# stella-cv/stella_vslam

Hardware: AMD Instinct MI355X
Metric: frames/s ORB-extract+match @640x480,2k kpts (higher is better)
Workload: dtype u8

## Files before the change

stella_vslam_amd/csrc/orb_kernels.hip:

```cpp
#include "svgpu_internal.h"
#include "sv_trig.h"
#include <utility>

#pragma clang fp contract(off)

namespace {

__device__ __constant__ float c_pattern_f[1024] = {
#include "orb_pattern_i8.inc"
};

__device__ __forceinline__ int find_level(const OrbLevel* __restrict__ L, int num_levels, int idx, int OrbLevel::*first,
                                          int* local) {
    int lv = 0;
    for (int l = 0; l < num_levels; ++l) {
        const int f = L[l].*first;
        if (idx >= f) lv = l;
    }
    *local = idx - L[lv].*first;
    return lv;
}

__device__ __forceinline__ int reflect101(int p, int len) {
    if (len == 1) return 0;
// ... 732 lines not shown
            const uint32_t order = (uint32_t)cell.order_base | ((uint32_t)ly << 7) | (uint32_t)qx;
            const unsigned long long key = ((unsigned long long)(uint32_t)s << 32) | (0xFFFFFFFFu - order);
            const int kx = gx - gx0, ky = gy - gy0;
            if ((unsigned)kx < FAST_KT && (unsigned)ky < FAST_KT) atomicMax(&s_key[ky * FAST_KT + kx], key);
            else atomicMax(&K[gy * lev.grid_x + gx], key);
        }
        if (found) atomicAdd(&s_count, found);
        __syncthreads();
        if (s_count > 0) break;
        __syncthreads();
    }
    }
    if (tid < FAST_KT * FAST_KT) {
        const unsigned long long key = s_key[tid];
        if (key) atomicMax(&K[(gy0 + tid / FAST_KT) * lev.grid_x + gx0 + tid % FAST_KT], key);
    }
    }
}

__global__ __launch_bounds__(1024) void k_select(const OrbLevel* __restrict__ L, int num_levels, unsigned long long* __restrict__ keys,
                                                 int total_grid, int4* __restrict__ sel, int32_t* __restrict__ counts, int32_t* __restrict__ cellpos) {
    __shared__ int s_wave[16], s_lvcnt[SV_MAX_LEVELS];
    const int b = blockIdx.x, tid = threadIdx.x, lane = tid & 63, wave = tid >> 6;
    unsigned long long* K = keys + (size_t)b * total_grid;
    int4* S = sel + (size_t)b * total_grid;
    if (tid < SV_MAX_LEVELS) s_lvcnt[tid] = 0;
    int running = 0;
    for (int base = 0; base < total_grid; base += 1024) {
        const int idx = base + tid;
        unsigned long long key = 0;
        if (idx < total_grid) {
            key = K[idx];
            if (key) K[idx] = 0;
        }
        const unsigned long long bal = __ballot(key != 0);
        const int before = __popcll(bal & ((1ull << lane) - 1ull));
        __syncthreads();
        if (lane == 0) s_wave[wave] = __popcll(bal);
        __syncthreads();
        int woff = 0, total = 0;
#pragma unroll
        for (int k = 0; k < 16; ++k) {
            if (k < wave) woff += s_wave[k];
            total += s_wave[k];
        }
        if (cellpos && idx < total_grid) cellpos[(size_t)b * (total_grid + 1) + idx] = running + woff + before;
        if (key) {
            int lv = 0;
            while (lv + 1 < num_levels && idx >= L[lv + 1].grid_first) ++lv;
            const uint32_t order = 0xFFFFFFFFu - (uint32_t)(key & 0xFFFFFFFFu);
            const int lx = order & 127, ly = (order >> 7) & 127, cid = order >> 14;
            const int cells_x = L[lv].cells_x;
            const int ci = cid / cells_x, cj = cid - ci * cells_x;
            int4 r;
            r.x = SV_PATCH_RADIUS + cj * SV_CELL + lx;
            r.y = SV_PATCH_RADIUS + ci * SV_CELL + ly;
            r.z = lv;
            r.w = (int)(key >> 32);
            S[running + woff + before] = r;
            atomicAdd(&s_lvcnt[lv], 1);
        }
        running += total;
    }
    __syncthreads();
    if (tid < num_levels) counts[b * (1 + num_levels) + 1 + tid] = s_lvcnt[tid];
    if (tid == 0) {
        counts[b * (1 + num_levels)] = running;
        if (cellpos) cellpos[(size_t)b * (total_grid + 1) + total_grid] = running;
    }
}

__device__ __forceinline__ float dev_fast_atan2(float y, float x) {
    const float p1 = 0.9997878412794807f * (float)(180 / 3.1415926535897932384626433832795);
    const float p3 = -0.3258083974640975f * (float)(180 / 3.1415926535897932384626433832795);
    const float p5 = 0.1555786518463281f * (float)(180 / 3.1415926535897932384626433832795);
    const float p7 = -0.04432655554792128f * (float)(180 / 3.1415926535897932384626433832795);
    const float eps = (float)2.2204460492503131e-16;
    const float ax = fabsf(x), ay = fabsf(y);
    float a, c, c2;
    if (ax >= ay) {
        c = ay / (ax + eps);
        c2 = c * c;
        a = (((p7 * c2 + p5) * c2 + p3) * c2 + p1) * c;
    }
    else {
        c = ax / (ay + eps);
        c2 = c * c;
        a = 90.f - (((p7 * c2 + p5) * c2 + p3) * c2 + p1) * c;
    }
    if (x < 0) a = 180.f - a;
    if (y < 0) a = 360.f - a;
    return a;
}

__device__ __forceinline__ float dev_util_cos(float v) { return sv_util_cos(v); }
__device__ __forceinline__ float dev_util_sin(float v) { return sv_util_sin(v); }

__device__ __forceinline__ int wave_sum(int v) {
    v += __builtin_amdgcn_update_dpp(0, v, 0x111, 0xF, 0xF, false);
    v += __builtin_amdgcn_update_dpp(0, v, 0x112, 0xF, 0xF, false);
    v += __builtin_amdgcn_update_dpp(0, v, 0x114, 0xF, 0xF, false);
    v += __builtin_amdgcn_update_dpp(0, v, 0x118, 0xF, 0xF, false);
    v += __builtin_amdgcn_update_dpp(0, v, 0x142, 0xA, 0xF, false);
    v += __builtin_amdgcn_update_dpp(0, v, 0x143, 0xC, 0xF, false);
    return __builtin_amdgcn_readlane(v, 63);
}

#ifndef DESC_KPW
#define DESC_KPW 5
#endif
#define DESC_IP 32
#define DESC_BP 40
#define DESC_R 18
#define DESC_SLAB (DESC_KPW * 37 * DESC_BP + 16)
struct IcWeights {
    uint32_t w1[256], wu[256];
};
constexpr IcWeights make_ic_weights() {
    constexpr int umax[16] = {15, 15, 15, 15, 14, 14, 14, 13, 13, 12, 11, 10, 9, 8, 6, 3};
    IcWeights t{};
    for (int row = 0; row < 31; ++row)
        for (int j = 0; j < 8; ++j) {
            uint32_t w1 = 0, wu = 0;
            const int v = row - 15, av = v < 0 ? -v : v;
            for (int k = 0; k < 4; ++k) {
                const int col = 4 * j + k, u = col - 15, au = u < 0 ? -u : u;
                if (col < 31 && au <= umax[av]) {
                    w1 |= 1u << (8 * k);
                    wu |= (uint32_t)(u + 15) << (8 * k);
                }
            }
            t.w1[row * 8 + j] = w1;
            t.wu[row * 8 + j] = wu;
        }
    return t;
}
__device__ __constant__ IcWeights c_icw = make_ic_weights();

__global__ __launch_bounds__(256) void k_describe(const OrbLevel* __restrict__ L, int num_levels, const int4* __restrict__ sel,
                                                  int total_grid, const int32_t* __restrict__ counts,
                                                  const uint8_t* __restrict__ img0, size_t img0_frame_stride, int img0_pitch,
                                                  const uint8_t* __restrict__ pyr, size_t pyr_frame_bytes,
                                                  const uint8_t* __restrict__ blur, size_t blur_frame_bytes,
                                                  svgpu_keypoint* __restrict__ kps, uint8_t* __restrict__ desc, int cap, float* __restrict__ angles) {
    __shared__ __attribute__((aligned(16))) uint8_t s_slab[4][DESC_SLAB];
    int b, blk;
    xcd_frame_map(gridDim.x, gridDim.y, blk, b);
    const int lane = threadIdx.x & 63, wave = __builtin_amdgcn_readfirstlane(threadIdx.x >> 6);
    const int n = min(counts[b * (1 + num_levels)], cap);
    const int i0 = (blk * 4 + wave) * DESC_KPW;
    if (i0 >= n) return;
    uint8_t* const slab = s_slab[wave];
    float px0[4], py0[4], px1[4], py1[4];
#pragma unroll
    for (int r = 0; r < 4; ++r) {
        const float4 q = reinterpret_cast<const float4*>(c_pattern_f)[r * 64 + lane];
        px0[r] = q.x;
        py0[r] = q.y;
        px1[r] = q.z;
        py1[r] = q.w;
    }
    uint32_t w1[4], wu[4];
    int rowv[4];
#pragma unroll
    for (int m = 0; m < 4; ++m) {
        const int item = lane + 64 * m;
        w1[m] = c_icw.w1[item];
        wu[m] = c_icw.wu[item];
        rowv[m] = (item >> 3) - 15;
    }
    const int nk = min(DESC_KPW, n - i0);
    const int4* const S = sel + (size_t)b * total_grid + i0;
    const uint8_t* const I0 = img0 + (size_t)b * img0_frame_stride;
    const uint8_t* const PY = pyr + (size_t)b * pyr_frame_bytes;
    const uint8_t* const BL = blur + (size_t)b * blur_frame_bytes;
    const int part = lane & 3, prow = lane >> 2;
    const int br = lane / 5, bpart = lane - 5 * br;
    int4 sv[DESC_KPW];
#pragma unroll
    for (int kk = 0; kk < DESC_KPW; ++kk) sv[kk] = S[kk];
    const uint8_t* gi[DESC_KPW];
    const uint8_t* gbl[DESC_KPW];
    int pit_i[DESC_KPW], pit_b[DESC_KPW];
#pragma unroll
    for (int kk = 0; kk < DESC_KPW; ++kk) {
        const int lv = kk < nk ? sv[kk].z : 0;
        pit_b[kk] = L[lv].pitch;
        pit_i[kk] = lv == 0 ? img0_pitch : pit_b[kk];
        gi[kk] = (lv == 0 ? I0 : PY + L[lv].pyr_off) + (size_t)(sv[kk].y - 15) * pit_i[kk] + (sv[kk].x - 15);
        gbl[kk] = BL + L[lv].blur_off + (size_t)(sv[kk].y - DESC_R) * pit_b[kk] + (sv[kk].x - DESC_R);
    }
    uint2 vi[DESC_KPW][2];
#pragma unroll
    for (int kk = 0; kk < DESC_KPW; ++kk)
        if (kk < nk) {
#pragma unroll
            for (int h = 0; h < 2; ++h)
                if (16 * h + prow < 31) __builtin_memcpy(&vi[kk][h], gi[kk] + (__umul24(16 * h + prow, pit_i[kk]) + 8 * part), 8);
        }
#pragma unroll
    for (int kk = 0; kk < DESC_KPW; ++kk)
        if (kk < nk) {
#pragma unroll
            for (int h = 0; h < 2; ++h)
                if (16 * h + prow < 31) *reinterpret_cast<uint2*>(slab + kk * (31 * DESC_IP) + (16 * h + prow) * DESC_IP + 8 * part) = vi[kk][h];
        }
    __builtin_amdgcn_fence(__ATOMIC_RELEASE, "wavefront");
    __builtin_amdgcn_wave_barrier();
    __builtin_amdgcn_fence(__ATOMIC_ACQUIRE, "wavefront");
    uint2 vb[DESC_KPW][4];
#pragma unroll
    for (int kk = 0; kk < DESC_KPW; ++kk)
        if (kk < nk) {
#pragma unroll
            for (int h = 0; h < 4; ++h)
                if (br < 12 && 12 * h + br < 37) __builtin_memcpy(&vb[kk][h], gbl[kk] + (__umul24(12 * h + br, pit_b[kk]) + 8 * bpart), 8);
        }
    int my10 = 0, my01 = 0;
#pragma unroll
    for (int kk = 0; kk < DESC_KPW; ++kk)
        if (kk < nk) {
            int m10 = 0, m01 = 0;
#pragma unroll
            for (int m = 0; m < 4; ++m) {
                const int item = lane + 64 * m;
                const uint32_t px = item < 248 ? reinterpret_cast<const uint32_t*>(slab + kk * (31 * DESC_IP))[item] : 0u;
                const int s1 = (int)__builtin_amdgcn_udot4(px, w1[m], 0u, false), su = (int)__builtin_amdgcn_udot4(px, wu[m], 0u, false);
                m10 += su - __mul24(15, s1);
                m01 += __mul24(rowv[m], s1);
            }
            m10 = wave_sum(m10);
            m01 = wave_sum(m01);
            if (lane == kk) {
                my10 = m10;
                my01 = m01;
            }
        }
    const float angle = dev_fast_atan2((float)my01, (float)my10);
    const float rad = (float)((double)angle * 3.14159265358979323846 / 180.0);
    const float ca_l = dev_util_cos(rad), sa_l = dev_util_sin(rad);
    __builtin_amdgcn_fence(__ATOMIC_RELEASE, "wavefront");
    __builtin_amdgcn_wave_barrier();
#pragma unroll
    for (int kk = 0; kk < DESC_KPW; ++kk)
        if (kk < nk) {
#pragma unroll
            for (int h = 0; h < 4; ++h)
                if (br < 12 && 12 * h + br < 37) *reinterpret_cast<uint2*>(slab + kk * (37 * DESC_BP) + __mul24(12 * h + br, DESC_BP) + 8 * bpart) = vb[kk][h];
        }
    __builtin_amdgcn_fence(__ATOMIC_RELEASE, "wavefront");
    __builtin_amdgcn_wave_barrier();
    __builtin_amdgcn_fence(__ATOMIC_ACQUIRE, "wavefront");
#pragma unroll
    for (int kk = 0; kk < DESC_KPW; ++kk)
        if (kk < nk) {
            const float ca = __int_as_float(__builtin_amdgcn_readlane(__float_as_int(ca_l), kk));
            const float sa = __int_as_float(__builtin_amdgcn_readlane(__float_as_int(sa_l), kk));
            const uint8_t* B = slab + kk * (37 * DESC_BP) + DESC_R * DESC_BP + DESC_R;
            unsigned long long bits[4];
#pragma unroll
            for (int r = 0; r < 4; ++r) {
                const float x0 = px0[r], y0 = py0[r], x1 = px1[r], y1 = py1[r];
                constexpr float RN = 12582912.0f;
                constexpr int RK = 0x400000 * DESC_BP + 0x4B400000;
                typedef float f32x2 __attribute__((ext_vector_type(2)));
                const f32x2 sc = {sa, ca}, cs = {ca, -sa}, rn = {RN, RN};
                const f32x2 q0 = (f32x2{x0, x0} * sc + f32x2{y0, y0} * cs) + rn;
                const f32x2 q1 = (f32x2{x1, x1} * sc + f32x2{y1, y1} * cs) + rn;
                const int r0 = __float_as_int(q0.x), c0 = __float_as_int(q0.y);
                const int r1 = __float_as_int(q1.x), c1 = __float_as_int(q1.y);
                const int a = B[__mul24(r0, DESC_BP) + c0 - RK];
                const int bb = B[__mul24(r1, DESC_BP) + c1 - RK];
                bits[r] = __builtin_amdgcn_ballot_w64(a < bb);
            }
            uint8_t* D = desc + ((size_t)b * cap + i0 + kk) * 32;
            if (lane < 4) reinterpret_cast<unsigned long long*>(D)[lane] = lane == 0 ? bits[0] : lane == 1 ? bits[1] : lane == 2 ? bits[2] : bits[3];
        }
    if (lane < nk) {
        const int4 s = S[lane];
        const int lv = s.z;
        svgpu_keypoint k;
        k.x = (float)s.x;
        k.y = (float)s.y;
        if (lv != 0) {
            k.x = k.x * L[lv].scale;
            k.y = k.y * L[lv].scale;
        }
        k.size = L[lv].kp_size;
        k.angle = angle;
        k.response = (float)s.w;
        k.octave = lv;
        k.class_id = -1;
        kps[(size_t)b * cap + i0 + lane] = k;
        if (angles) angles[(size_t)b * cap + i0 + lane] = angle;
    }
}


#ifndef DB_THREADS
#define DB_THREADS 512
#endif
#define DB_WAVES (DB_THREADS / 64)
#define DB_MAX_KP 128
struct IcWeights3 {
    uint32_t w1[256], wu[256], wv[256];
};
constexpr IcWeights3 make_ic_weights3() {
    constexpr int umax[16] = {15, 15, 15, 15, 14, 14, 14, 13, 13, 12, 11, 10, 9, 8, 6, 3};
    IcWeights3 t{};
    for (int row = 0; row < 31; ++row)
        for (int j = 0; j < 8; ++j) {
            uint32_t w1 = 0, wu = 0, wv = 0;
            const int v = row - 15, av = v < 0 ? -v : v;
            for (int k = 0; k < 4; ++k) {
                const int col = 4 * j + k, u = col - 15, au = u < 0 ? -u : u;
                if (col < 31 && au <= umax[av]) {
                    w1 |= 1u << (8 * k);
                    wu |= (uint32_t)(u + 15) << (8 * k);
                    wv |= (uint32_t)row << (8 * k);
                }
            }
            t.w1[row * 8 + j] = w1;
            t.wu[row * 8 + j] = wu;
            t.wv[row * 8 + j] = wv;
        }
    return t;
}
__device__ __constant__ IcWeights3 c_icw3 = make_ic_weights3();

template <int LANE>
__device__ __forceinline__ void sv_writelane8(uint32_t& lo, uint32_t& hi, const unsigned long long (&m)[4]) {
    asm("s_nop 1\n\tv_writelane_b32 %0, %2, %10\n\tv_writelane_b32 %1, %3, %10\n\tv_writelane_b32 %0, %4, %11\n\tv_writelane_b32 %1, %5, %11\n\t"
        "v_writelane_b32 %0, %6, %12\n\tv_writelane_b32 %1, %7, %12\n\tv_writelane_b32 %0, %8, %13\n\tv_writelane_b32 %1, %9, %13"
        : "+v"(lo), "+v"(hi)
        : "s"((uint32_t)m[0]), "s"((uint32_t)(m[0] >> 32)), "s"((uint32_t)m[1]), "s"((uint32_t)(m[1] >> 32)), "s"((uint32_t)m[2]), "s"((uint32_t)(m[2] >> 32)),
          "s"((uint32_t)m[3]), "s"((uint32_t)(m[3] >> 32)), "n"(LANE), "n"(LANE + 1), "n"(LANE + 2), "n"(LANE + 3));
}

__device__ __forceinline__ void db_stage_rows(const uint8_t* img, int gp, int y0, int nrows, int cpr, uint32_t lds0, int lane, int wave) {
    const int rpi = 64 / cpr;
    const int rsub = lane / cpr, csub = lane - rsub * cpr;
    const uint32_t voff = (uint32_t)(rsub * gp + csub * 16);
    const int groups = (nrows + rpi - 1) / rpi;
    const unsigned long long base = (unsigned long long)(uintptr_t)(img + (size_t)y0 * gp);
    if (rsub < rpi)
        for (int g = wave; g < groups; g += DB_WAVES)
            if (g * rpi + rsub < nrows) sv_glds16(base + (unsigned long long)(g * rpi) * (unsigned)gp, voff, lds0 + (uint32_t)(g * rpi * cpr) * 16);
}
__device__ __forceinline__ void db_stage_rows_wide(const uint8_t* img, int gp, int y0, int nrows, int cpr, uint32_t lds0, int lane, int wave) {
    const int total = nrows * cpr;
    int q = wave * 64 + lane;
    int row = q / cpr, c = q - row * cpr;
    const int drow = (DB_WAVES * 64) / cpr, dc = (DB_WAVES * 64) - drow * cpr;
    const unsigned long long base = (unsigned long long)(uintptr_t)(img + (size_t)y0 * gp);
    uint32_t dst = lds0 + wave * 1024;
    for (int i = wave * 64; i < total; i += DB_WAVES * 64) {
        if (q < total) sv_glds16(base, (uint32_t)(row * gp + c * 16), dst);
        q += DB_WAVES * 64;
        row += drow;
        c += dc;
        if (c >= cpr) {
            c -= cpr;
            ++row;
        }
        dst += DB_WAVES * 1024;
    }
}

__global__ __launch_bounds__(DB_THREADS) void k_describe_bands(const OrbLevel* __restrict__ L, int num_levels, const DescBand* __restrict__ bands, int num_bands,
                                                               const int4* __restrict__ sel, int total_grid, const int32_t* __restrict__ cellpos,
                                                               const int32_t* __restrict__ counts,
                                                               const uint8_t* __restrict__ img0, size_t img0_frame_stride, int img0_pitch,
                                                               const uint8_t* __restrict__ pyr, size_t pyr_frame_bytes,
                                                               const uint8_t* __restrict__ blur, size_t blur_frame_bytes,
                                                               svgpu_keypoint* __restrict__ kps, uint8_t* __restrict__ desc, int cap, float* __restrict__ angles) {
    extern __shared__ __attribute__((aligned(16))) uint8_t s_band[];
    int b, bi;
    xcd_frame_map(gridDim.x, gridDim.y, bi, b);
    const DescBand bd = bands[bi];
    const int tid = threadIdx.x, lane = tid & 63, wave = __builtin_amdgcn_readfirstlane(tid >> 6);
    const int32_t* const P = cellpos + (size_t)b * (total_grid + 1);
    const int n = min(counts[b * (1 + num_levels)], cap);
    const int p0 = P[bd.cell0], nkp = min(P[bd.cell1], n) - p0;
    if (nkp <= 0) return;
    const int lv = bd.lv, lp = bd.lp, cpr = lp >> 4;
    int2* const s_xy = reinterpret_cast<int2*>(s_band + bd.img_bytes);
    int2* const s_aux = s_xy + DB_MAX_KP;
    const uint32_t lds0 = __builtin_amdgcn_readfirstlane((uint32_t)(uintptr_t)(const __attribute__((address_space(3))) uint8_t*)s_band);
    const int4* const S = sel + (size_t)b * total_grid + p0;
    int4 sv = make_int4(0, 0, 0, 0);
    if (tid < nkp) {
        sv = S[tid];
        s_xy[tid] = make_int2(sv.x, sv.y);
    }
    uint32_t w1[4], wu[4], wv[4];
#pragma unroll
    for (int m = 0; m < 4; ++m) {
        const int item = lane + 64 * m;
        w1[m] = c_icw3.w1[item];
        wu[m] = c_icw3.wu[item];
        wv[m] = c_icw3.wv[item];
    }
    float px0[4], py0[4], px1[4], py1[4];
#pragma unroll
    for (int r = 0; r < 4; ++r) {
        const float4 q = reinterpret_cast<const float4*>(c_pattern_f)[r * 64 + lane];
        px0[r] = q.x;
        py0[r] = q.y;
        px1[r] = q.z;
        py1[r] = q.w;
    }
    {
        const uint8_t* img = lv == 0 ? img0 + (size_t)b * img0_frame_stride : pyr + (size_t)b * pyr_frame_bytes + L[lv].pyr_off;
        asm volatile("s_waitcnt vmcnt(0) lgkmcnt(0)" ::: "memory");
        if (cpr <= 64) db_stage_rows(img, lv == 0 ? img0_pitch : L[lv].pitch, bd.yu0, bd.nru, cpr, lds0, lane, wave);
        else db_stage_rows_wide(img, lv == 0 ? img0_pitch : L[lv].pitch, bd.yu0, bd.nru, cpr, lds0, lane, wave);
        asm volatile("s_waitcnt vmcnt(0)" ::: "memory");
    }
    __syncthreads();
    {
        const int lane_off = (lane >> 3) * lp + 4 * (lane & 7), step = 8 * lp;
        for (int j = wave; j < nkp; j += DB_WAVES) {
            const int2 xy = s_xy[j];
            const int x = __builtin_amdgcn_readfirstlane(xy.x), y = __builtin_amdgcn_readfirstlane(xy.y);
            const int org = (y - 15 - bd.yu0) * lp + (x - 15);
            const uint32_t* U = reinterpret_cast<const uint32_t*>(s_band + ((org & ~3) + lane_off));
            const uint32_t sh = (org & 3) * 8;
            uint32_t s1 = 0, su = 0, sw = 0;
#pragma unroll
            for (int m = 0; m < 4; ++m) {
                const uint32_t lo = U[m * (step >> 2)], hi = U[m * (step >> 2) + 1];
                const uint32_t px = __builtin_amdgcn_alignbit(hi, lo, sh);
                s1 = __builtin_amdgcn_udot4(px, w1[m], s1, false);
                su = __builtin_amdgcn_udot4(px, wu[m], su, false);
                sw = __builtin_amdgcn_udot4(px, wv[m], sw, false);
            }
            const int m10 = wave_sum((int)su - __mul24(15, (int)s1)), m01 = wave_sum((int)sw - __mul24(15, (int)s1));
            if (lane == 0) s_aux[j] = make_int2(m10, m01);
        }
    }
    __syncthreads();
    if (cpr <= 64) db_stage_rows(blur + (size_t)b * blur_frame_bytes + L[lv].blur_off, L[lv].pitch, bd.yb0, bd.nrb, cpr, lds0, lane, wave);
    else db_stage_rows_wide(blur + (size_t)b * blur_frame_bytes + L[lv].blur_off, L[lv].pitch, bd.yb0, bd.nrb, cpr, lds0, lane, wave);
    if (tid < nkp) {
        const int2 mm = s_aux[tid];
        const float angle = dev_fast_atan2((float)mm.y, (float)mm.x);
        const float rad = (float)((double)angle * 3.14159265358979323846 / 180.0);
        s_aux[tid] = make_int2(__float_as_int(dev_util_cos(rad)), __float_as_int(dev_util_sin(rad)));
        svgpu_keypoint k;
        k.x = (float)sv.x;
        k.y = (float)sv.y;
        if (lv != 0) {
            k.x = k.x * L[lv].scale;
            k.y = k.y * L[lv].scale;
        }
        k.size = L[lv].kp_size;
        k.angle = angle;
        k.response = (float)sv.w;
        k.octave = lv;
        k.class_id = -1;
        kps[(size_t)b * cap + p0 + tid] = k;
        if (angles) angles[(size_t)b * cap + p0 + tid] = angle;
    }
    asm volatile("s_waitcnt vmcnt(0)" ::: "memory");
    __syncthreads();
    {
        constexpr float RN = 12582912.0f;
        const int rk = 0x400000 * lp + 0x4B400000;
        for (int j = wave; j < nkp; j += DB_WAVES) {
            const int2 xy = s_xy[j], cs2 = s_aux[j];
            const int x = __builtin_amdgcn_readfirstlane(xy.x), y = __builtin_amdgcn_readfirstlane(xy.y);
            const float ca = __int_as_float(__builtin_amdgcn_readfirstlane(cs2.x)), sa = __int_as_float(__builtin_amdgcn_readfirstlane(cs2.y));
            const uint8_t* B = s_band + ((y - bd.yb0) * lp + x - rk);
            unsigned long long bits[4];
#pragma unroll
            for (int r = 0; r < 4; ++r) {
                typedef float f32x2 __attribute__((ext_vector_type(2)));
                const f32x2 sc = {sa, ca}, cs = {ca, -sa}, rn = {RN, RN};
                const f32x2 q0 = (f32x2{px0[r], px0[r]} * sc + f32x2{py0[r], py0[r]} * cs) + rn;
                const f32x2 q1 = (f32x2{px1[r], px1[r]} * sc + f32x2{py1[r], py1[r]} * cs) + rn;
                const int a = B[__mul24(__float_as_int(q0.x), lp) + __float_as_int(q0.y)];
                const int bb = B[__mul24(__float_as_int(q1.x), lp) + __float_as_int(q1.y)];
                bits[r] = __builtin_amdgcn_ballot_w64(a < bb);
            }
            uint32_t d_lo = 0, d_hi = 0;
            sv_writelane8<0>(d_lo, d_hi, bits);
            if (lane < 4) reinterpret_cast<uint2*>(desc + ((size_t)b * cap + p0 + j) * 32)[lane] = make_uint2(d_lo, d_hi);
        }
    }
}

}

hipError_t sv_pyramid_prepare() {
    return sv_allow_dynamic_lds(reinterpret_cast<const void*>(k_pyramid_lds), SV_PYR_LDS_MAX);
}
void sv_launch_pyramid(hipStream_t s, const OrbFrames& F, const OrbLaunch& plan, const int2* band_rows, int bands, size_t lds_bytes, const short* xofs,
                       const short2* xa, const short2* yofs, const short2* yb, const uint32_t* xg, const short4* yrow) {
    if (plan.pyramid_lds)
        hipLaunchKernelGGL(k_pyramid_lds, dim3(bands, F.batch), dim3(PYR_THREADS), lds_bytes, s, F.levels, F.num_levels, band_rows, bands, F.img0,
                           F.img0_frame_stride, F.img0_pitch, F.pyr, F.pyr_frame_bytes, xg, yrow);
    else
        hipLaunchKernelGGL(k_pyramid, dim3(bands, F.batch), dim3(PYR_THREADS), 0, s, F.levels, F.num_levels, band_rows, F.img0, F.img0_frame_stride,
                           F.img0_pitch, F.pyr, F.pyr_frame_bytes, xofs, xa, yofs, yb);
}

void sv_launch_blur(hipStream_t s, const OrbFrames& F, const OrbLaunch& plan, int total_tiles, int total_bands) {
    const dim3 grid(total_tiles, F.batch), block(256);
    if (!plan.blur_bands) {
        hipLaunchKernelGGL(k_blur<BLUR_ROWS_SMALL>, grid, block, 0, s, F.levels, F.num_levels, F.img0, F.img0_frame_stride, F.img0_pitch, F.pyr,
                           F.pyr_frame_bytes, F.blur, F.blur_frame_bytes);
        if (plan.need_gather)
            hipLaunchKernelGGL(k_blur_gather<BLUR_ROWS_SMALL>, grid, block, 0, s, F.levels, F.num_levels, F.img0, F.img0_frame_stride, F.img0_pitch, F.pyr,
                               F.pyr_frame_bytes, F.blur, F.blur_frame_bytes);
    }
    else {
        hipLaunchKernelGGL(k_blur<BLUR_ROWS>, dim3(total_bands, F.batch), dim3(BLUR_BAND_THREADS), 0, s, F.levels, F.num_levels, F.img0, F.img0_frame_stride,
                           F.img0_pitch, F.pyr, F.pyr_frame_bytes, F.blur, F.blur_frame_bytes);
        if (plan.need_gather)
            hipLaunchKernelGGL(k_blur_gather<BLUR_ROWS>, grid, block, 0, s, F.levels, F.num_levels, F.img0, F.img0_frame_stride, F.img0_pitch, F.pyr,
                               F.pyr_frame_bytes, F.blur, F.blur_frame_bytes);
    }
}

void sv_launch_fast(hipStream_t s, const OrbFrames& F, int cpw, const FastCell* cells, int num_cells, const unsigned short* gtab,
                    unsigned long long* keys, int total_grid, int ini_thr, int min_thr, const uint8_t* mask, size_t mask_frame_stride,
                    int mask_pitch, int mask_w, int mask_h) {
    if (num_cells == 0) return;
    hipLaunchKernelGGL(k_fast, dim3((num_cells + cpw - 1) / cpw, F.batch), dim3(256), 0, s, F.levels, F.num_levels, cells, num_cells, cpw, F.img0,
                       F.img0_frame_stride, F.img0_pitch, F.pyr, F.pyr_frame_bytes, gtab, keys, total_grid, ini_thr, min_thr, mask, mask_frame_stride,
                       mask_pitch, mask_w, mask_h);
}

void sv_launch_select(hipStream_t s, const OrbFrames& F, unsigned long long* keys, int total_grid, int4* sel, int32_t* counts, int32_t* cellpos) {
    hipLaunchKernelGGL(k_select, dim3(F.batch), dim3(1024), 0, s, F.levels, F.num_levels, keys, total_grid, sel, counts, cellpos);
}

void sv_launch_describe(hipStream_t s, const OrbFrames& F, const int4* sel, int total_grid, const int32_t* counts, svgpu_keypoint* kps,
                        uint8_t* desc, int cap, float* angles) {
    if (total_grid == 0) return;
    hipLaunchKernelGGL(k_describe, dim3((total_grid + 4 * DESC_KPW - 1) / (4 * DESC_KPW), F.batch), dim3(256), 0, s, F.levels, F.num_levels, sel, total_grid,
                       counts, F.img0, F.img0_frame_stride, F.img0_pitch, F.pyr, F.pyr_frame_bytes, F.blur, F.blur_frame_bytes, kps, desc, cap, angles);
}

hipError_t sv_describe_bands_prepare(size_t lds_bytes) {
    return sv_allow_dynamic_lds(reinterpret_cast<const void*>(k_describe_bands), lds_bytes);
}
void sv_launch_describe_bands(hipStream_t s, const OrbFrames& F, const DescBand* bands, int num_bands, size_t lds_bytes, const int4* sel,
                              int total_grid, const int32_t* cellpos, const int32_t* counts, svgpu_keypoint* kps, uint8_t* desc, int cap,
                              float* angles) {
    if (num_bands == 0) return;
    hipLaunchKernelGGL(k_describe_bands, dim3(num_bands, F.batch), dim3(DB_THREADS), lds_bytes, s, F.levels, F.num_levels, bands, num_bands, sel, total_grid,
                       cellpos, counts, F.img0, F.img0_frame_stride, F.img0_pitch, F.pyr, F.pyr_frame_bytes, F.blur, F.blur_frame_bytes, kps, desc, cap, angles);
}
```

Before: 283,900.

## Process multiple keypoints per wave in intensity centroid and preload per-lane keypoint data

The intensity-centroid phase now splits each wave into groups (two keypoints per wave by default), each group reducing with DPP row shifts instead of a full wave_sum. The third weight table (row weights) is dropped: m01 is reconstructed from a running prefix sum of s1 per row, removing one udot4 per iteration and one constant array. The descriptor phase loads each wave's keypoint coordinates and cos/sin once into lanes and extracts them with readlane per iteration, instead of an LDS load per keypoint. This shortens the serial per-keypoint latency chain at the cost of more complex indexing and reliance on DPP row semantics and on the DB_MAX_KP/DB_WAVES assumptions.

Result: no change. 285,900, median of 6 (+0.7%).

```diff
diff --git a/stella_vslam_amd/csrc/orb_kernels.hip b/stella_vslam_amd/csrc/orb_kernels.hip
--- a/stella_vslam_amd/csrc/orb_kernels.hip
+++ b/stella_vslam_amd/csrc/orb_kernels.hip
@@ -1058,27 +1058,43 @@
 #endif
 #define DB_WAVES (DB_THREADS / 64)
 #define DB_MAX_KP 128
+#ifndef DB_KPG
+#define DB_KPG 2
+#endif
+#define DB_GL (64 / DB_KPG)
+#define DB_GR (DB_GL / 8)
+#define DB_GI (32 / DB_GR)
+static_assert(DB_KPG == 1 || DB_KPG == 2 || DB_KPG == 4, "a group is one, two or four DPP rows");
+static_assert(DB_MAX_KP % DB_WAVES == 0 && (DB_MAX_KP / DB_WAVES & (DB_MAX_KP / DB_WAVES - 1)) == 0 && DB_MAX_KP / DB_WAVES <= 64,
+              "phase B keeps a wave's keypoints one per lane");
+__device__ __forceinline__ int db_group_sum(int v) {
+    v += __builtin_amdgcn_update_dpp(0, v, 0x111, 0xF, 0xF, false);
+    v += __builtin_amdgcn_update_dpp(0, v, 0x112, 0xF, 0xF, false);
+    v += __builtin_amdgcn_update_dpp(0, v, 0x114, 0xF, 0xF, false);
+    v += __builtin_amdgcn_update_dpp(0, v, 0x118, 0xF, 0xF, false);
+    if (DB_GL >= 32) v += __builtin_amdgcn_update_dpp(0, v, 0x142, 0xA, 0xF, false);
+    if (DB_GL == 64) v += __builtin_amdgcn_update_dpp(0, v, 0x143, 0xC, 0xF, false);
+    return v;
+}
 struct IcWeights3 {
-    uint32_t w1[256], wu[256], wv[256];
+    uint32_t w1[256], wu[256];
 };
 constexpr IcWeights3 make_ic_weights3() {
     constexpr int umax[16] = {15, 15, 15, 15, 14, 14, 14, 13, 13, 12, 11, 10, 9, 8, 6, 3};
     IcWeights3 t{};
     for (int row = 0; row < 31; ++row)
         for (int j = 0; j < 8; ++j) {
-            uint32_t w1 = 0, wu = 0, wv = 0;
+            uint32_t w1 = 0, wu = 0;
             const int v = row - 15, av = v < 0 ? -v : v;
             for (int k = 0; k < 4; ++k) {
                 const int col = 4 * j + k, u = col - 15, au = u < 0 ? -u : u;
                 if (col < 31 && au <= umax[av]) {
                     w1 |= 1u << (8 * k);
                     wu |= (uint32_t)(u + 15) << (8 * k);
-                    wv |= (uint32_t)row << (8 * k);
                 }
             }
             t.w1[row * 8 + j] = w1;
             t.wu[row * 8 + j] = wu;
-            t.wv[row * 8 + j] = wv;
         }
     return t;
 }
@@ -1149,13 +1165,13 @@
         sv = S[tid];
         s_xy[tid] = make_int2(sv.x, sv.y);
     }
-    uint32_t w1[4], wu[4], wv[4];
-#pragma unroll
-    for (int m = 0; m < 4; ++m) {
-        const int item = lane + 64 * m;
+    const int gl = lane & (DB_GL - 1), r0 = gl >> 3;
+    uint32_t w1[DB_GI], wu[DB_GI];
+#pragma unroll
+    for (int m = 0; m < DB_GI; ++m) {
+        const int item = (r0 + DB_GR * m) * 8 + (lane & 7);
         w1[m] = c_icw3.w1[item];
         wu[m] = c_icw3.wu[item];
-        wv[m] = c_icw3.wv[item];
     }
     float px0[4], py0[4], px1[4], py1[4];
 #pragma unroll
@@ -1175,24 +1191,25 @@
     }
     __syncthreads();
     {
-        const int lane_off = (lane >> 3) * lp + 4 * (lane & 7), step = 8 * lp;
-        for (int j = wave; j < nkp; j += DB_WAVES) {
-            const int2 xy = s_xy[j];
-            const int x = __builtin_amdgcn_readfirstlane(xy.x), y = __builtin_amdgcn_readfirstlane(xy.y);
-            const int org = (y - 15 - bd.yu0) * lp + (x - 15);
+        const int lane_off = r0 * lp + 4 * (lane & 7), step = DB_GR * lp, grp = lane / DB_GL;
+        for (int j0 = wave * DB_KPG; j0 < nkp; j0 += DB_WAVES * DB_KPG) {
+            const int j = j0 + grp;
+            const int2 xy = s_xy[min(j, nkp - 1)];
+            const int org = (xy.y - 15 - bd.yu0) * lp + (xy.x - 15);
             const uint32_t* U = reinterpret_cast<const uint32_t*>(s_band + ((org & ~3) + lane_off));
             const uint32_t sh = (org & 3) * 8;
-            uint32_t s1 = 0, su = 0, sw = 0;
-#pragma unroll
-            for (int m = 0; m < 4; ++m) {
+            uint32_t s1 = 0, su = 0, sb = 0;
+#pragma unroll
+            for (int m = DB_GI - 1; m >= 0; --m) {
                 const uint32_t lo = U[m * (step >> 2)], hi = U[m * (step >> 2) + 1];
                 const uint32_t px = __builtin_amdgcn_alignbit(hi, lo, sh);
                 s1 = __builtin_amdgcn_udot4(px, w1[m], s1, false);
                 su = __builtin_amdgcn_udot4(px, wu[m], su, false);
-                sw = __builtin_amdgcn_udot4(px, wv[m], sw, false);
-            }
-            const int m10 = wave_sum((int)su - __mul24(15, (int)s1)), m01 = wave_sum((int)sw - __mul24(15, (int)s1));
-            if (lane == 0) s_aux[j] = make_int2(m10, m01);
+                sb += s1;
+            }
+            const int m10 = db_group_sum((int)su - __mul24(15, (int)s1));
+            const int m01 = db_group_sum(__mul24(DB_GR, (int)sb) + __mul24(r0 - DB_GR - 15, (int)s1));
+            if (gl == DB_GL - 1 && j < nkp) s_aux[j] = make_int2(m10, m01);
         }
     }
     __syncthreads();
@@ -1223,10 +1240,12 @@
     {
         constexpr float RN = 12582912.0f;
         const int rk = 0x400000 * lp + 0x4B400000;
-        for (int j = wave; j < nkp; j += DB_WAVES) {
-            const int2 xy = s_xy[j], cs2 = s_aux[j];
-            const int x = __builtin_amdgcn_readfirstlane(xy.x), y = __builtin_amdgcn_readfirstlane(xy.y);
-            const float ca = __int_as_float(__builtin_amdgcn_readfirstlane(cs2.x)), sa = __int_as_float(__builtin_amdgcn_readfirstlane(cs2.y));
+        const int jl = min(wave + DB_WAVES * (lane & (DB_MAX_KP / DB_WAVES - 1)), nkp - 1);
+        const int2 xyl = s_xy[jl], csl = s_aux[jl];
+        int i = 0;
+        for (int j = wave; j < nkp; j += DB_WAVES, ++i) {
+            const int x = __builtin_amdgcn_readlane(xyl.x, i), y = __builtin_amdgcn_readlane(xyl.y, i);
+            const float ca = __int_as_float(__builtin_amdgcn_readlane(csl.x, i)), sa = __int_as_float(__builtin_amdgcn_readlane(csl.y, i));
             const uint8_t* B = s_band + ((y - bd.yb0) * lp + x - rk);
             unsigned long long bits[4];
 #pragma unroll
```
